# zhizdev/sparsefusion

Hardware: AMD Instinct MI355X
Metric: novel views/sec, distillation steps (2 NGP renders fwd+bwd + VAE enc/dec + 51-eval PLMS + LPIPS), 256^2 / 32x32 latents, 2-view synthetic hydrant (higher is better)
Workload: dtype bf16 MFMA operands / f32 accumulate (UNet); f32 (NGP render)

## Files before the change

include/sparsefusion_hip.h:

```cpp
#ifndef SPARSEFUSION_HIP_H
#define SPARSEFUSION_HIP_H

#include <stdint.h>

#ifdef __cplusplus
extern "C" {
#endif

#define SF_OK 0
#define SF_ERR_INVALID 1
#define SF_ERR_LAUNCH 2

const char* sf_last_error(void);
int sf_abi_version(void);
int sf_operand_is_f16(void);


int sf_grid_encode_forward(const float* inputs, const float* embeddings,
                           const int32_t* offsets, float* outputs,
                           uint32_t B, uint32_t D, uint32_t C, uint32_t L,
                           float S, uint32_t H, float* dy_dx,
                           uint32_t gridtype, int align_corners,
                           const int32_t* h_offsets, void* stream);

// ... 104 lines not shown
int sf_mc_count(const float* vol, uint32_t nx, uint32_t ny, uint32_t nz, float iso,
                void* workspace, uint64_t workspace_bytes, uint32_t* counts2, void* stream);
int sf_mc_emit(const float* vol, uint32_t nx, uint32_t ny, uint32_t nz, float iso,
               void* workspace, uint64_t workspace_bytes, float* verts, int32_t* faces,
               void* stream);

int sf_ngp_render_forward(const sf_ngp_field* f, const float* rays_o,
                          const float* rays_d, const float* aabb, uint32_t N,
                          uint32_t T, float min_near, const float* lin,
                          const float* u_coarse, const float* u_fine,
                          uint32_t u_fine_row_stride, float bg_color, float* nears,
                          float* fars, float* z_sorted, float* sigma_s,
                          float* rgb_s, float* image, float* depth,
                          float* weights_sum, float* field_cache, float* workspace,
                          uint64_t workspace_bytes, void* stream);

int sf_ngp_render_backward(const sf_ngp_field* f, const sf_ngp_field_grad* g,
                           const float* rays_o, const float* rays_d,
                           const float* aabb, uint32_t N, uint32_t T,
                           const float* nears, const float* fars,
                           const float* z_sorted, const float* sigma_s,
                           const float* rgb_s, float bg_color,
                           const float* grad_image, const float* grad_weights_sum,
                           uint32_t rays_per_row, const float* field_cache,
                           float* workspace, uint64_t workspace_bytes,
                           void* stream);

uint64_t sf_ngp_render_workspace_bytes(uint32_t N, uint32_t T);
uint64_t sf_ngp_render_forward_workspace_bytes(uint32_t N, uint32_t T);

uint64_t sf_ngp_render_cache_bytes(uint32_t N, uint32_t T);

int sf_ngp_field_mfma(int on);

int sf_ngp_render_shaded_forward(const sf_ngp_field* f, const float* rays_o, const float* rays_d, const float* aabb,
                                 uint32_t N, uint32_t T, float min_near, const float* lin, const float* u_coarse,
                                 const float* u_fine, uint32_t u_fine_row_stride, float bg_color, const float* light_d,
                                 float ambient_ratio, float epsilon, float* nears, float* fars, float* z_sorted,
                                 float* sigma_s, float* rgb_s, float* normal_s, float* rgb_shaded_s, float* xyz_s,
                                 float* image, float* normal_image, float* orient, float* depth, float* weights_sum,
                                 float* workspace, uint64_t workspace_bytes, void* stream);
uint64_t sf_ngp_render_shaded_workspace_bytes(uint32_t N, uint32_t T);

int sf_ngp_render_occ_eval(const sf_ngp_field* f, const float* rays_o, const float* rays_d,
                           const float* nears, const float* fars, const uint8_t* grid,
                           float dt_gamma, uint32_t max_steps, uint32_t C, uint32_t H,
                           const float* noises, float T_thresh, uint32_t N,
                           float* weights_sum, float* depth, float* image, void* stream);

int sf_ngp_render_occ_eval_shaded(const sf_ngp_field* f, const float* rays_o, const float* rays_d,
        const float* nears, const float* fars, const uint8_t* grid, float dt_gamma, uint32_t max_steps,
        uint32_t C, uint32_t H, const float* noises, float T_thresh, uint32_t N,
        const float* light_d , float ambient_ratio, float epsilon,
        float* weights_sum, float* depth, float* image,
        float* normal_image , uint32_t* n_samples ,
        void* stream);


enum {
  SF_OP_CONV = 1,
  SF_OP_GN_ACT = 2,
  SF_OP_LN = 3,
  SF_OP_GEMV = 4,
  SF_OP_ATTN = 5,
  SF_OP_GCA_POOL = 6,
  SF_OP_ELTWISE = 7,
// ... 81 lines not shown
```

sparsefusion_amd/_lib.py:

```python
import ctypes as C
import os

import torch

_HERE = os.path.dirname(os.path.abspath(__file__))
_DEFAULT_LIB = "libsparsefusion_hip_f16.so" if os.environ.get("SF_OPERAND", "bf16").lower() in ("f16", "fp16", "half") else "libsparsefusion_hip.so"
LIB_PATH = os.environ.get("SF_HIP_LIB") or os.path.join(_HERE, _DEFAULT_LIB)

_lib = None

c_f32p = C.c_void_p
c_i32p = C.c_void_p
u32 = C.c_uint32
u64 = C.c_uint64


class SfNgpField(C.Structure):
    _fields_ = [("embeddings", C.c_void_p), ("h_offsets", C.c_void_p), ("L", u32), ("S", C.c_float),
                ("H", u32), ("gridtype", u32),
                ("w0", C.c_void_p), ("b0", C.c_void_p), ("w1", C.c_void_p), ("b1", C.c_void_p),
                ("w2", C.c_void_p), ("b2", C.c_void_p), ("bound", C.c_float)]


class SfNgpFieldGrad(C.Structure):
# ... 45 lines not shown
                                C.c_void_p, c_f32p, c_f32p, c_f32p, c_f32p, c_f32p, c_f32p, C.c_void_p]),
    "sf_composite_rays": (C.c_int, [u32, u32, C.c_float, c_i32p, c_f32p, c_f32p, c_f32p, c_f32p, c_f32p, c_f32p,
                                    c_f32p, C.c_void_p]),
    "sf_adam_multi": (C.c_int, [C.POINTER(SfAdamArgs), C.c_void_p]),
    "sf_loss_partial_rows": (u32, []),
    "sf_upsample2x_forward": (C.c_int, [c_f32p, c_f32p, u32, u32, u32, C.c_void_p]),
    "sf_upsample2x_backward": (C.c_int, [c_f32p, c_f32p, u32, u32, u32, C.c_void_p]),
    "sf_render_loss_forward": (C.c_int, [c_f32p, c_f32p, c_f32p, c_f32p, u64, u64, C.c_float, c_f32p, C.c_void_p]),
    "sf_render_loss_backward": (C.c_int, [c_f32p, c_f32p, c_f32p, c_f32p, u64, u64, C.c_float, C.c_float, C.c_float, C.c_float,
                                          C.c_float, c_f32p, c_f32p, c_f32p, C.c_void_p]),
    "sf_fusion_loss_forward": (C.c_int, [c_f32p, c_f32p, c_f32p, c_f32p, u32, u64, u64, c_f32p, C.c_void_p]),
    "sf_fusion_loss_backward": (C.c_int, [c_f32p, c_f32p, c_f32p, c_f32p, u32, u64, u64, C.c_float, C.c_float, C.c_float,
                                          c_f32p, c_f32p, c_f32p, C.c_void_p]),
    "sf_ngp_density": (C.c_int, [C.POINTER(SfNgpField), c_f32p, u32, c_f32p, c_f32p, C.c_void_p]),
    "sf_ngp_density_lattice": (C.c_int, [C.POINTER(SfNgpField), c_f32p, c_f32p, c_f32p, u32, u32, u32, c_f32p, C.c_void_p]),
    "sf_ngp_point_attrs": (C.c_int, [C.POINTER(SfNgpField), c_f32p, u32, C.c_float, c_f32p, c_f32p, c_f32p, c_f32p, C.c_void_p]),
    "sf_ngp_texture_bake": (C.c_int, [C.POINTER(SfNgpField), c_f32p, u32, c_i32p, u32, u32, C.c_void_p, c_f32p, c_f32p, c_i32p,
                                      C.c_void_p]),
    "sf_gaussian3d_workspace_bytes": (u64, [u32, u32, u32]),
    "sf_gaussian3d": (C.c_int, [c_f32p, c_f32p, u32, u32, u32, C.c_float, C.c_float, C.c_void_p, C.c_void_p, u64, C.c_void_p]),
    "sf_mc_workspace_bytes": (u64, [u32, u32, u32]),
    "sf_mc_count": (C.c_int, [c_f32p, u32, u32, u32, C.c_float, C.c_void_p, u64, C.c_void_p, C.c_void_p]),
    "sf_mc_emit": (C.c_int, [c_f32p, u32, u32, u32, C.c_float, C.c_void_p, u64, c_f32p, c_i32p, C.c_void_p]),
    "sf_ngp_render_forward": (C.c_int, [C.POINTER(SfNgpField), c_f32p, c_f32p, c_f32p, u32, u32, C.c_float,
                                        c_f32p, c_f32p, c_f32p, u32, C.c_float, c_f32p, c_f32p, c_f32p, c_f32p,
                                        c_f32p, c_f32p, c_f32p, c_f32p, c_f32p, c_f32p, u64, C.c_void_p]),
    "sf_ngp_render_backward": (C.c_int, [C.POINTER(SfNgpField), C.POINTER(SfNgpFieldGrad), c_f32p, c_f32p,
                                         c_f32p, u32, u32, c_f32p, c_f32p, c_f32p, c_f32p, c_f32p,
                                         C.c_float, c_f32p, c_f32p, u32, c_f32p, c_f32p, u64, C.c_void_p]),
    "sf_ngp_render_workspace_bytes": (u64, [u32, u32]),
    "sf_ngp_render_forward_workspace_bytes": (u64, [u32, u32]),
    "sf_ngp_render_cache_bytes": (u64, [u32, u32]),
    "sf_ngp_field_mfma": (C.c_int, [C.c_int]),
    "sf_ngp_render_shaded_forward": (C.c_int, [C.POINTER(SfNgpField), c_f32p, c_f32p, c_f32p, u32, u32, C.c_float, c_f32p, c_f32p,
                                               c_f32p, u32, C.c_float, c_f32p, C.c_float, C.c_float, c_f32p, c_f32p, c_f32p,
                                               c_f32p, c_f32p, c_f32p, c_f32p, c_f32p, c_f32p, c_f32p, c_f32p, c_f32p, c_f32p,
                                               c_f32p, u64, C.c_void_p]),
    "sf_ngp_render_shaded_workspace_bytes": (u64, [u32, u32]),
    "sf_ngp_render_occ_eval": (C.c_int, [C.POINTER(SfNgpField), c_f32p, c_f32p, c_f32p, c_f32p, C.c_void_p, C.c_float, u32, u32, u32,
                                         c_f32p, C.c_float, u32, c_f32p, c_f32p, c_f32p, C.c_void_p]),
    "sf_ngp_render_occ_eval_shaded": (C.c_int, [C.POINTER(SfNgpField), c_f32p, c_f32p, c_f32p, c_f32p, C.c_void_p, C.c_float, u32, u32,
                                                u32, c_f32p, C.c_float, u32, c_f32p, C.c_float, C.c_float, c_f32p, c_f32p, c_f32p,
                                                c_f32p, C.c_void_p, C.c_void_p]),
    "sf_plan_run": (C.c_int, [C.POINTER(SfOp), u32, C.c_void_p]),
    "sf_conv_igemm_t_launches": (u64, []),
    "sf_gca4_launches": (u64, [C.c_int]),
    "sf_plan_profile": (C.c_int, [C.POINTER(SfOp), u32, C.c_void_p, C.c_void_p]),
    "sf_conv_packed_elems": (u64, [u32, u32, u32, u32]),
    "sf_conv_pack_weights": (C.c_int, [C.c_void_p, u32, u32, u32, u32, u32, C.c_void_p]),
    "sf_plms_update": (C.c_int, [c_f32p, c_f32p, c_f32p, C.c_void_p, u64, c_f32p, c_f32p, C.c_void_p]),
    "sf_plms_combine": (C.c_int, [c_f32p, c_f32p, c_f32p, c_f32p, C.c_void_p, u64, c_f32p, c_f32p, C.c_void_p]),
    "sf_plms_step": (C.c_int, [c_f32p, c_f32p, c_f32p, c_f32p, C.c_void_p, c_f32p, c_f32p, c_f32p, C.c_void_p, u64, c_f32p, c_f32p, c_f32p, u64, C.c_void_p]),
}


_handles = {}


def _load(path):
    if path not in _handles:
        if not os.path.exists(path):
            raise RuntimeError(
                f"{path} is missing: build it with `python -m sparsefusion_amd.build` (`--f16` for the IEEE-half operand build; "
                "there is no CPU fallback for the sparsefusion_amd hot path)")
        handle = C.CDLL(path)
        for name, (res, args) in SIGNATURES.items():
# ... 43 lines not shown
```

sparsefusion_amd/csrc/ngp_render.hip:

```cpp

#include "sf_common.h"
#include "ngp_device.h"
#include "ngp_field_lds.h"
#include "ngp_bwd_mfma.h"
#include "ngp_field_mfma.h"
#include "ngp_composite_wave.h"
#include "ngp_scatter_bin.h"
#include "ngp_shade.h"
#include <stdlib.h>
#include <atomic>
#include <mutex>

struct GridLevels;
int sf_fill_levels(GridLevels* lv, const int32_t* offsets_dev, const int32_t* h_offsets, uint32_t L, float S,
                   uint32_t H, hipStream_t st);

template <int MODE>
__global__ __launch_bounds__(256) void k_ngp_field(
    FieldPtrs f, NgpLevels lv, const float* __restrict__ rays_o, const float* __restrict__ rays_d,
    const float* __restrict__ aabb, const float* __restrict__ nears, const float* __restrict__ fars,
    const float* __restrict__ lin, const float* __restrict__ u, const float* __restrict__ z_in,
    const float* __restrict__ xyz_in, uint32_t P, uint32_t T, float* __restrict__ z_out,
    float* __restrict__ sigma, float* __restrict__ rgb, float* __restrict__ feat_out = nullptr) {
  __shared__ __attribute__((aligned(16))) float W[NGP_WTOTAL];
  load_weights_lds(W, f);
  __syncthreads();
  float box[6];
  if (MODE != 2) {
#pragma unroll
    for (int i = 0; i < 6; ++i) box[i] = aabb[i];
  }
  for (uint32_t p = blockIdx.x * blockDim.x + threadIdx.x; p < P; p += gridDim.x * blockDim.x) {
    asm volatile("" ::: "memory");
    float x[3];
    if (MODE == 2) {
      x[0] = xyz_in[p * 3 + 0]; x[1] = xyz_in[p * 3 + 1]; x[2] = xyz_in[p * 3 + 2];
    } else {
// ... 246 lines not shown
    uint32_t per = 8192;
    if ((N + per - 1) / per > 64) per = (((N + 63) / 64 + 255) / 256) * 256;
    c.n = (N + per - 1) / per; c.max_rays = per;
    for (uint32_t i = 0; i < c.n; ++i) c.start[i] = i * per;
    c.start[c.n] = N;
    return c;
  }
  equal(k);
  return c;
}
#define SB_CURSOR_WORDS (NGP_MAX_LEVELS * SB_MAX_BUCKETS)
#ifndef SB_LEVELS_BUDGET
#define SB_LEVELS_BUDGET 24
#endif
static uint64_t ngp_bin_entries(uint32_t N, uint32_t T) {
  return (uint64_t)ngp_bwd_plan(N).max_rays * 2 * T * 4 * SB_LEVELS_BUDGET + (uint64_t)SB_CURSOR_WORDS * 64;
}
extern "C" uint64_t sf_ngp_render_workspace_bytes(uint32_t N, uint32_t T) {
  return (uint64_t)(8 + 4 * NGP_MAX_LEVELS) * N * T * sizeof(float) + (uint64_t)SB_CURSOR_WORDS * 4 + ngp_bin_entries(N, T) * 16;
}

extern "C" uint64_t sf_ngp_render_forward_workspace_bytes(uint32_t N, uint32_t T) { return (uint64_t)10 * N * T * sizeof(float); }

#ifndef FM_GRID_CAP
#define FM_GRID_CAP 512u
#endif
static std::atomic<int> g_field_mfma{1};
extern "C" int sf_ngp_field_mfma(int on) {
  const int was = g_field_mfma.load(std::memory_order_relaxed);
  if (on >= 0) g_field_mfma.store(on ? 1 : 0, std::memory_order_relaxed);
  return was;
}

extern "C" uint64_t sf_ngp_render_cache_bytes(uint32_t N, uint32_t T) {
  return ((uint64_t)2 * N * T * NGP_FEAT + (uint64_t)N * 2 * T) * sizeof(float);
}

extern "C" int sf_ngp_render_forward(const sf_ngp_field* f, const float* rays_o, const float* rays_d,
                                     const float* aabb, uint32_t N, uint32_t T, float min_near,
                                     const float* lin, const float* u_coarse, const float* u_fine,
                                     uint32_t u_fine_row_stride, float bg_color, float* nears, float* fars,
                                     float* z_sorted, float* sigma_s, float* rgb_s, float* image, float* depth,
                                     float* weights_sum, float* field_cache, float* workspace, uint64_t workspace_bytes,
                                     void* stream) {
  hipStream_t st = (hipStream_t)stream;
  if (N == 0) return SF_OK;
  if (T < 4 || T > 64) SF_FAIL(SF_ERR_INVALID, "ngp_render: T must be in [4,64]");
  if (workspace_bytes < sf_ngp_render_forward_workspace_bytes(N, T)) SF_FAIL(SF_ERR_INVALID, "ngp_render: workspace too small");
  if (!lin || !u_fine) SF_FAIL(SF_ERR_INVALID, "ngp_render: lin and u_fine tables are required");
  NgpLevels lv;
  if (int rc = sf_ngp_make_levels(f, &lv, st)) return rc;
  if (int rc = sf_near_far_from_aabb(rays_o, rays_d, aabb, N, min_near, nears, fars, stream)) return rc;
  const uint64_t NT = (uint64_t)N * T;
  float* z_c = workspace;           float* sig_c = z_c + NT;     float* rgb_c = sig_c + NT;
  float* z_f = rgb_c + 3 * NT;      float* sig_f = z_f + NT;     float* rgb_f = sig_f + NT;
  const FieldPtrs fp = field_ptrs(f);
  const uint32_t P = (uint32_t)NT;
  const uint32_t gridp = sf_grid_cap(sf_div_up(P, 256));
  float* feat_c = field_cache;
  float* feat_f = field_cache ? field_cache + NT * NGP_FEAT : nullptr;
  uint32_t* perm = field_cache ? reinterpret_cast<uint32_t*>(field_cache + 2 * NT * NGP_FEAT) : nullptr;
  const bool mfma = g_field_mfma.load(std::memory_order_relaxed) != 0;
  FMArgs fm{};
  fm.table = fp.table; fm.w0 = fp.w0; fm.b0 = fp.b0; fm.w1 = fp.w1; fm.b1 = fp.b1; fm.w2 = fp.w2; fm.b2 = fp.b2; fm.bound = fp.bound;
  fm.lv = lv; fm.rays_o = rays_o; fm.rays_d = rays_d; fm.aabb = aabb; fm.nears = nears; fm.fars = fars; fm.P = P; fm.T = T;
  const uint32_t gridm = sf_div_up(sf_div_up(P, FM_PTS), 4) < FM_GRID_CAP ? sf_div_up(sf_div_up(P, FM_PTS), 4) : FM_GRID_CAP;
// ... 106 lines not shown
      props.allocType = hipMemAllocationTypePinned;
      props.location.type = hipMemLocationTypeDevice;
      props.location.id = dev_id;
      hipMemPool_t np = nullptr;
      uint64_t keep = UINT64_MAX;
      if (hipMemPoolCreate(&np, &props) != hipSuccess) SF_FAIL(SF_ERR_LAUNCH, "ngp_render_backward: cannot create the scratch pool");
      if (hipMemPoolSetAttribute(np, hipMemPoolAttrReleaseThreshold, &keep) != hipSuccess) {
        (void)hipMemPoolDestroy(np);
        SF_FAIL(SF_ERR_LAUNCH, "ngp_render_backward: cannot configure the scratch pool");
      }
      pools[dev_id] = np;
    }
    pool = pools[dev_id];
  }
  struct FixBuf {
    long long* p = nullptr; hipStream_t st = nullptr;
    ~FixBuf() { if (p) (void)hipFreeAsync(p, st); }
  } fix;
  fix.st = st;
  const uint64_t fix_bytes = segs.end[FIX_SEGS - 1] * sizeof(long long);
  const hipError_t alloc = pool ? hipMallocFromPoolAsync(reinterpret_cast<void**>(&fix.p), fix_bytes, pool, st)
                               : hipMallocAsync(reinterpret_cast<void**>(&fix.p), fix_bytes, st);
  if (alloc != hipSuccess || !fix.p)
    SF_FAIL(SF_ERR_LAUNCH, "ngp_render_backward: cannot allocate the gradient accumulators");
  if (hipMemsetAsync(fix.p, 0, fix_bytes, st) != hipSuccess) SF_FAIL(SF_ERR_LAUNCH, "ngp_render_backward: memset failed");
  long long* acc_tab = fix.p;
  long long* acc_mlp = fix.p + tab_n;
  const float thr_tab = sf_fix_thr(8.0 * (double)M);
  const size_t lds2 = (size_t)FB_LDS_FLOATS * sizeof(float);
  const size_t lds_sc = (size_t)SC_SLOTS * (sizeof(uint32_t) + 2 * sizeof(long long));
  static unsigned attr_mask = 0;
  if (dev_id >= 32 || !(attr_mask & (1u << dev_id))) {
    if (hipFuncSetAttribute(reinterpret_cast<const void*>(&k_ngp_field_bwd_mfma), hipFuncAttributeMaxDynamicSharedMemorySize, (int)lds2) != hipSuccess ||
        hipFuncSetAttribute(reinterpret_cast<const void*>(&k_ngp_scatter<1024>), hipFuncAttributeMaxDynamicSharedMemorySize, (int)lds_sc) != hipSuccess)
      SF_FAIL(SF_ERR_LAUNCH, "ngp_render_backward: cannot raise the dynamic LDS limits");
    if (dev_id < 32) attr_mask |= 1u << dev_id;
  }
  constexpr float sc_cutoff = 640.0f;
#ifndef SC_RUN
#define SC_RUN 32u
#endif
  constexpr uint32_t sc_run = SC_RUN;
  uint32_t cached = 0;
  while (cached < lv.L && lv.scale[cached] <= sc_cutoff) ++cached;
  constexpr float bin_cutoff = 60.0f;
  uint32_t first_bin = lv.L;
  uint32_t bucket0[NGP_MAX_LEVELS + 1] = {};
  if (dfeat) {
    first_bin = 0;
    while (first_bin < lv.L && lv.scale[first_bin] <= bin_cutoff) ++first_bin;
    uint32_t tb = 0;
    for (uint32_t l = 0; l <= NGP_MAX_LEVELS; ++l) {
      bucket0[l] = tb;
      if (l >= first_bin && l < lv.L) {
        const uint32_t nb = (lv.hsize[l] + SB_ROWS - 1) >> SB_ROWS_LOG;
        if (nb > SB_MAX_BUCKETS) { first_bin = lv.L; break; }
        tb += nb;
      }
    }
  }
  const bool binned = first_bin < lv.L;
  if (binned && cached > first_bin) cached = first_bin;
  const uint32_t last = !dfeat ? lv.L : binned ? first_bin : cached;
  const uint32_t total_buckets = bucket0[NGP_MAX_LEVELS];
  uint32_t* bin_cursor = reinterpret_cast<uint32_t*>(workspace + (size_t)(8 + 4 * NGP_MAX_LEVELS) * N * T);
  f32x4* bin_ent = reinterpret_cast<f32x4*>(bin_cursor + SB_CURSOR_WORDS);
// ... 12 lines not shown
  std::unique_lock<std::mutex> side_lk(side_mu, std::defer_lock);
  struct SideJoin {
    Side* sd = nullptr; hipStream_t st = nullptr; bool forked = false;
    int join() { const bool f = forked; forked = false; return (!f || (hipEventRecord(sd->join, sd->s) == hipSuccess && hipStreamWaitEvent(st, sd->join, 0) == hipSuccess)) ? 0 : 1; }
    ~SideJoin() { (void)join(); }
  } side_join;
  if (fork) {
    side_lk.lock();
    Side& sd = side[dev_id];
    if (!sd.s && (hipStreamCreateWithFlags(&sd.s, hipStreamNonBlocking) != hipSuccess ||
                  hipEventCreateWithFlags(&sd.fork, hipEventDisableTiming) != hipSuccess ||
                  hipEventCreateWithFlags(&sd.join, hipEventDisableTiming) != hipSuccess))
      SF_FAIL(SF_ERR_LAUNCH, "ngp_render_backward: cannot create the side stream");
    side_join.sd = &sd; side_join.st = st;
  }
  const uint32_t T2 = 2 * T;
  for (uint32_t c = 0; c < n_chunks; ++c) {
    const uint32_t n0 = plan.start[c], Nc = plan.start[c + 1] - n0;
    const uint32_t Pc = Nc * T2, P0 = n0 * T2;
    FBArgs a{};
    a.table = f->embeddings; a.w0 = f->w0; a.b0 = f->b0; a.w1 = f->w1; a.b1 = f->b1; a.w2 = f->w2; a.b2 = f->b2; a.bound = f->bound;
    a.g_w0 = acc_mlp + (segs.end[0] - tab_n); a.g_b0 = acc_mlp + (segs.end[1] - tab_n); a.g_w1 = acc_mlp + (segs.end[2] - tab_n);
    a.g_b1 = acc_mlp + (segs.end[3] - tab_n); a.g_w2 = acc_mlp + (segs.end[4] - tab_n); a.g_b2 = acc_mlp + (segs.end[5] - tab_n);
    a.f_w0 = g->g_w0; a.f_b0 = g->g_b0; a.f_w1 = g->g_w1; a.f_b1 = g->g_b1; a.f_w2 = g->g_w2; a.f_b2 = g->g_b2; a.thr = thr_mlp;
    a.lv = lv;
    a.rays_o = rays_o + (size_t)n0 * 3; a.rays_d = rays_d + (size_t)n0 * 3; a.aabb = aabb;
    a.z_s = z_sorted + (size_t)P0; a.dsig = dsig + (size_t)P0; a.drgb = drgb + (size_t)P0 * 3; a.dfeat_out = dfeat;
    a.P = Pc; a.T2 = T2; a.dfeat_P = (uint32_t)M; a.p_off = P0;
    a.feat_c = field_cache;
    a.feat_f = field_cache ? field_cache + (size_t)N * T * NGP_FEAT : nullptr;
    a.perm = field_cache ? reinterpret_cast<const uint32_t*>(field_cache + 2 * (size_t)N * T * NGP_FEAT) : nullptr;
    const uint32_t trips = sf_div_up(Pc, FB_PTS);
    const uint32_t grid = trips < 1024 ? sf_div_up(trips, 4) : 256;
    k_ngp_field_bwd_mfma<<<grid, 256, lds2, st>>>(a);
    SF_CHECK_LAUNCH("ngp_field_bwd_mfma");
    if (dfeat && last < lv.L) {
      hipStream_t sf = st;
      if (fork) {
        Side& sd = side[dev_id];
        if (hipEventRecord(sd.fork, st) != hipSuccess || hipStreamWaitEvent(sd.s, sd.fork, 0) != hipSuccess)
          SF_FAIL(SF_ERR_LAUNCH, "ngp_render_backward: fork failed");
        sf = sd.s;
        side_join.forked = true;
      }
      if (binned) {
        SBArgs b{};
        b.lv = lv; b.bound = f->bound; b.rays_o = a.rays_o; b.rays_d = a.rays_d; b.aabb = aabb; b.z_s = a.z_s; b.dfeat = dfeat;
        b.gtable = acc_tab; b.gtable_f = g->g_embeddings; b.thr = thr_tab; b.cursor = bin_cursor; b.ent = bin_ent;
        b.P = Pc; b.T2 = T2; b.first_level = first_bin; b.P_stride = (uint32_t)M; b.p_off = P0; b.cap = bin_cap;
        SBRArgs r{};
        r.lv = lv; r.gtable = acc_tab; r.gtable_f = g->g_embeddings; r.thr = thr_tab; r.cursor = bin_cursor; r.ent = bin_ent; r.first_level = first_bin; r.cap = bin_cap;
        for (uint32_t l = 0; l <= NGP_MAX_LEVELS; ++l) { b.bucket0[l] = bucket0[l]; r.bucket0[l] = bucket0[l]; }
        const uint32_t tiles = sf_div_up(Pc, SB_THREADS);
        k_ngp_bin<<<tiles < 1024 ? tiles : 1024, SB_THREADS, 0, sf>>>(b);
        SF_CHECK_LAUNCH("ngp_bin");
        k_ngp_bin_reduce<<<total_buckets, SBR_THREADS, 0, sf>>>(r);
        SF_CHECK_LAUNCH("ngp_bin_reduce");
      } else {
        const uint64_t items = (uint64_t)4 * Pc * (lv.L - last);
        const uint32_t grid_f = (uint32_t)(items / 256 < 16384 ? (items + 255) / 256 : 16384);
        k_ngp_scatter_fine<<<grid_f, 256, 0, sf>>>(lv, f->bound, acc_tab, g->g_embeddings, thr_tab, a.rays_o, a.rays_d, aabb, a.z_s, dfeat, Nc, T2, last,
                                                   (uint32_t)M, P0);
        SF_CHECK_LAUNCH("ngp_scatter_fine");
      }
    }
  }
  if (dfeat && last > 0) {
    const uint32_t grid_sc = sf_div_up(N, SC_RAYS);
// ... 13 lines not shown
```

sparsefusion_amd/nerf/renderer.py:

```python
import argparse
import ctypes as C
import math
import os

import torch
import torch.nn as nn

from .. import _lib
from .utils import safe_normalize


def get_default_torch_ngp_opt():
    opt = argparse.Namespace()
    opt.cuda_ray = False
    opt.max_steps = 256
    opt.num_steps = 64
    opt.upsample_steps = 64
    opt.update_extra_interval = 16
    opt.max_ray_batch = 4096
    opt.albedo_iters = 1000
    opt.bg_radius = 0
    opt.density_thresh = 10
    opt.fp16 = True
    opt.backbone = 'grid'
# ... 6 lines not shown
    opt.lambda_entropy = 1e-4
    opt.lambda_opacity = 0
    opt.lambda_orient = 1e-2
    opt.lambda_smooth = 0
    return opt


class _FieldHandle:

    def __init__(self, net):
        enc = net.encoder
        lin = net.sigma_net.net
        self.tensors = [enc.embeddings, lin[0].weight, lin[0].bias, lin[1].weight, lin[1].bias, lin[2].weight,
                        lin[2].bias]
        self.host_offsets = enc.host_offsets
        self.L = enc.num_levels
        self.S = float(math.log2(enc.per_level_scale))
        self.H = int(enc.base_resolution)
        self.gridtype = int(enc.gridtype_id)
        self.bound = float(net.bound)

    def struct(self, tensors):
        f = _lib.SfNgpField()
        f.embeddings = tensors[0].data_ptr()
        f.h_offsets = self.host_offsets.ctypes.data
        f.L, f.S, f.H, f.gridtype = self.L, self.S, self.H, self.gridtype
        f.w0, f.b0, f.w1, f.b1, f.w2, f.b2 = (t.data_ptr() for t in tensors[1:])
        f.bound = self.bound
        return f


_FEAT_CACHE = True
_FIELD_MFMA = True


def _select_field_kernel(lib):
    lib.sf_ngp_field_mfma(1 if _FIELD_MFMA else 0)


class _RenderFn(torch.autograd.Function):
    @staticmethod
    def forward(ctx, handle, rays_o, rays_d, aabb, T, min_near, lin, u_coarse, u_fine, u_stride, bg, rays_per_row, grad_mode, *params):
        _lib.require_cuda(rays_o, rays_d, aabb, *params)
        params = [p.detach().contiguous() for p in params]
        N = rays_o.shape[0]
        dev = rays_o.device
        f32 = dict(dtype=torch.float32, device=dev)
        nears, fars = torch.empty(N, **f32), torch.empty(N, **f32)
        z_s, sig_s = torch.empty(N, 2 * T, **f32), torch.empty(N, 2 * T, **f32)
        rgb_s = torch.empty(N, 2 * T, 3, **f32)
        image, depth, ws = torch.empty(N, 3, **f32), torch.empty(N, **f32), torch.empty(N, **f32)
        lib = _lib.lib()
        wbytes = lib.sf_ngp_render_forward_workspace_bytes(N, T)
        work = torch.empty(max(1, wbytes // 4), **f32)
        f = handle.struct(params)
        cache = None
        if _FEAT_CACHE and grad_mode and any(ctx.needs_input_grad[13:]):
            cache = torch.empty(lib.sf_ngp_render_cache_bytes(N, T) // 4, **f32)
        _select_field_kernel(lib)
        rc = lib.sf_ngp_render_forward(C.byref(f), _lib.ptr(rays_o), _lib.ptr(rays_d), _lib.ptr(aabb), N, T,
                                       float(min_near), _lib.ptr(lin), _lib.ptr(u_coarse), _lib.ptr(u_fine),
                                       int(u_stride), float(bg), _lib.ptr(nears), _lib.ptr(fars), _lib.ptr(z_s),
                                       _lib.ptr(sig_s), _lib.ptr(rgb_s), _lib.ptr(image), _lib.ptr(depth), _lib.ptr(ws),
                                       _lib.ptr(cache), _lib.ptr(work), wbytes, _lib.stream_ptr())
        _lib.check(rc, "ngp_render_forward")
        ctx.handle, ctx.T, ctx.bg, ctx.rays_per_row = handle, T, float(bg), int(rays_per_row)
        ctx.has_cache = cache is not None
        ctx.save_for_backward(rays_o, rays_d, aabb, nears, fars, z_s, sig_s, rgb_s, *([cache] if cache is not None else []), *params)
        ctx.mark_non_differentiable(depth, nears, fars)
        return image, ws, depth, nears, fars

    @staticmethod
    def backward(ctx, g_image, g_ws, _gd, _gn, _gf):
        rays_o, rays_d, aabb, nears, fars, z_s, sig_s, rgb_s, *params = ctx.saved_tensors
        cache = params.pop(0) if ctx.has_cache else None
        N, T = rays_o.shape[0], ctx.T
        grads = [torch.zeros_like(p) for p in params]
        g = _lib.SfNgpFieldGrad()
        (g.g_embeddings, g.g_w0, g.g_b0, g.g_w1, g.g_b1, g.g_w2, g.g_b2) = (t.data_ptr() for t in grads)
        f = ctx.handle.struct(params)
        lib = _lib.lib()
        wbytes = lib.sf_ngp_render_workspace_bytes(N, T)
        work = torch.empty(max(1, wbytes // 4), dtype=torch.float32, device=rays_o.device)
        g_image = (g_image if g_image is not None else torch.zeros(N, 3, device=rays_o.device)).contiguous().float()
        g_ws = g_ws.contiguous().float() if g_ws is not None else None
        rc = lib.sf_ngp_render_backward(C.byref(f), C.byref(g), _lib.ptr(rays_o), _lib.ptr(rays_d), _lib.ptr(aabb), N, T,
                                        _lib.ptr(nears), _lib.ptr(fars), _lib.ptr(z_s), _lib.ptr(sig_s), _lib.ptr(rgb_s),
                                        ctx.bg, _lib.ptr(g_image), _lib.ptr(g_ws), int(ctx.rays_per_row), _lib.ptr(cache),
                                        _lib.ptr(work), wbytes, _lib.stream_ptr())
        _lib.check(rc, "ngp_render_backward")
        return (None,) * 13 + tuple(grads)


class NeRFRenderer(nn.Module):
    def __init__(self, opt):
        super().__init__()
        self.opt = opt
        self.bound = opt.bound
        self.cascade = 1 + math.ceil(math.log2(opt.bound))
        self.grid_size = 128
        self.cuda_ray = opt.cuda_ray
        self.min_near = opt.min_near
        self.density_thresh = opt.density_thresh
        self.bg_radius = opt.bg_radius
        if self.bg_radius > 0:
            raise NotImplementedError("bg_radius > 0 is not on the distillation path (distillation.py:512)")
        box = torch.tensor([-opt.bound] * 3 + [opt.bound] * 3, dtype=torch.float32)
        self.register_buffer('aabb_train', box)
        self.register_buffer('aabb_infer', box.clone())
        self._tables = {}
        if self.cuda_ray:
            self.register_buffer('density_grid', torch.zeros([self.cascade, self.grid_size ** 3]))
            self.register_buffer('density_bitfield', torch.zeros(self.cascade * self.grid_size ** 3 // 8, dtype=torch.uint8))
            self.mean_density = 0
            self.iter_density = 0
            self.register_buffer('step_counter', torch.zeros(16, 2, dtype=torch.int32))
            self.mean_count = 0
            self.local_step = 0
# ... 321 lines not shown
```

Baseline: 18.29.

## Add software-pipelined NGP field backward kernel with prefetch and register-resident weights

Result: faster. 18.52 (median of 6 runs) (+1.2%).

```diff
diff --git a/include/sparsefusion_hip.h b/include/sparsefusion_hip.h
--- a/include/sparsefusion_hip.h
+++ b/include/sparsefusion_hip.h
@@ -160,6 +160,9 @@
 uint64_t sf_ngp_render_cache_bytes(uint32_t N, uint32_t T);
 
 int sf_ngp_field_mfma(int on);
+
+int sf_ngp_field_bwd_pipe(int on);
+void sf_ngp_field_bwd_launches(uint64_t* counts);
 
 int sf_ngp_render_shaded_forward(const sf_ngp_field* f, const float* rays_o, const float* rays_d, const float* aabb,
                                  uint32_t N, uint32_t T, float min_near, const float* lin, const float* u_coarse,
diff --git a/sparsefusion_amd/_lib.py b/sparsefusion_amd/_lib.py
--- a/sparsefusion_amd/_lib.py
+++ b/sparsefusion_amd/_lib.py
@@ -101,6 +101,8 @@
     "sf_ngp_render_forward_workspace_bytes": (u64, [u32, u32]),
     "sf_ngp_render_cache_bytes": (u64, [u32, u32]),
     "sf_ngp_field_mfma": (C.c_int, [C.c_int]),
+    "sf_ngp_field_bwd_pipe": (C.c_int, [C.c_int]),
+    "sf_ngp_field_bwd_launches": (None, [C.c_void_p]),
     "sf_ngp_render_shaded_forward": (C.c_int, [C.POINTER(SfNgpField), c_f32p, c_f32p, c_f32p, u32, u32, C.c_float, c_f32p, c_f32p,
                                                c_f32p, u32, C.c_float, c_f32p, C.c_float, C.c_float, c_f32p, c_f32p, c_f32p,
                                                c_f32p, c_f32p, c_f32p, c_f32p, c_f32p, c_f32p, c_f32p, c_f32p, c_f32p, c_f32p,
diff --git a/sparsefusion_amd/csrc/ngp_bwd_pipe.h b/sparsefusion_amd/csrc/ngp_bwd_pipe.h
--- /dev/null
+++ b/sparsefusion_amd/csrc/ngp_bwd_pipe.h
@@ -0,0 +1,433 @@
+#pragma once
+#include "ngp_bwd_mfma.h"
+
+#ifndef SF_FIELD_BWD_PIPE_DEFAULT
+#define SF_FIELD_BWD_PIPE_DEFAULT 1
+#endif
+#ifndef FP_W1_REGS
+#define FP_W1_REGS 1
+#endif
+#ifndef FP_H1_REGS
+#define FP_H1_REGS 1
+#endif
+#ifndef FP_PREFETCH
+#define FP_PREFETCH 1
+#endif
+
+struct FPOps {
+  f32x4 fv[4];
+  float z, o[3], d[3];
+  float g0, g1;
+};
+
+SF_DEV void fp_load(const FBArgs& a, uint32_t pc, uint32_t src, int half, FPOps& q) {
+  const uint32_t pg = a.p_off + pc, ng = pg / a.T2, T = a.T2 >> 1, n = pc / a.T2;
+  const float* row = (src < T ? a.feat_c + ((size_t)ng * T + src) * NGP_FEAT : a.feat_f + ((size_t)ng * T + (src - T)) * NGP_FEAT) + half * 16;
+#pragma unroll
+  for (int j = 0; j < 4; ++j) q.fv[j] = *reinterpret_cast<const f32x4*>(row + 4 * j);
+  q.z = a.z_s[pc];
+#pragma unroll
+  for (int i = 0; i < 3; ++i) { q.o[i] = a.rays_o[n * 3 + i]; q.d[i] = a.rays_d[n * 3 + i]; }
+  q.g0 = half == 0 ? a.dsig[pc] : a.drgb[(size_t)pc * 3 + 1];
+  q.g1 = half == 0 ? a.drgb[(size_t)pc * 3] : a.drgb[(size_t)pc * 3 + 2];
+}
+
+SF_KERNEL(256) void k_ngp_field_bwd_pipe(FBArgs a) {
+  SF_DYN_LDS(lds_raw);
+  float* W = reinterpret_cast<float*>(lds_raw);
+  const int tid = threadIdx.x, lane = tid & 63, wave = tid >> 6;
+  float* F = W + FB_WTOT + wave * FB_WAVE_FLOATS;
+  float* H1 = F + FB_PTS * FB_SF;
+  float* H2 = H1 + FB_PTS * FB_SH;
+  float* DO = H2 + FB_PTS * FB_SH;
+  float* INS = DO + FB_PTS * 4;
+  for (int i = tid; i < NGP_HID * NGP_FEAT; i += 256) W[FB_W0 + (i >> 5) * FB_SF + (i & 31)] = a.w0[i];
+  for (int i = tid; i < NGP_HID * NGP_HID; i += 256) W[FB_W1 + (i >> 6) * FB_SH + (i & 63)] = a.w1[i];
+  for (int i = tid; i < NGP_OUT * NGP_HID; i += 256) W[FB_W2 + i] = a.w2[i];
+  if (tid < NGP_HID) { W[FB_B0 + tid] = a.b0[tid]; W[FB_B1 + tid] = a.b1[tid]; }
+  if (tid < NGP_OUT) W[FB_B2 + tid] = a.b2[tid];
+  float box[6];
+#pragma unroll
+  for (int i = 0; i < 6; ++i) box[i] = a.aabb[i];
+  sf_sync();
+
+  const int li = lane & 15, kq = lane >> 4;
+  const int pl = lane & 31, half = lane >> 5;
+#if FP_W1_REGS >= 1
+  float bw1[NGP_HID / 4][4];
+#pragma unroll
+  for (int s = 0; s < NGP_HID / 4; ++s)
+#pragma unroll
+    for (int nt = 0; nt < 4; ++nt) bw1[s][nt] = W[FB_W1 + (nt * 16 + li) * FB_SH + 4 * s + kq];
+#endif
+#if FP_W1_REGS >= 2
+  float gw1[NGP_HID / 4][4];
+#pragma unroll
+  for (int s = 0; s < NGP_HID / 4; ++s)
+#pragma unroll
+    for (int nt = 0; nt < 4; ++nt) gw1[s][nt] = W[FB_W1 + (4 * s + kq) * FB_SH + nt * 16 + li];
+#endif
+  float cw2[NGP_HID / 4], ew2[4], bb0[4], bb1[4];
+#pragma unroll
+  for (int s = 0; s < NGP_HID / 4; ++s) {
+    const float v = W[FB_W2 + (li & 3) * NGP_HID + 4 * s + kq];
+    cw2[s] = li < NGP_OUT ? v : 0.0f;
+  }
+#pragma unroll
+  for (int nt = 0; nt < 4; ++nt) {
+    ew2[nt] = W[FB_W2 + kq * NGP_HID + nt * 16 + li];
+    bb0[nt] = W[FB_B0 + nt * 16 + li];
+    bb1[nt] = W[FB_B1 + nt * 16 + li];
+  }
+  const float cb2 = li < NGP_OUT ? W[FB_B2 + (li & 3)] : 0.0f;
+
+  f32x4 acc1[4][4], acc0[4][2];
+  f32x4 acc2[4], accb2 = f32x4{0.f, 0.f, 0.f, 0.f};
+#pragma unroll
+  for (int i = 0; i < 4; ++i) {
+#pragma unroll
+    for (int j = 0; j < 4; ++j) acc1[i][j] = f32x4{0.f, 0.f, 0.f, 0.f};
+    acc0[i][0] = f32x4{0.f, 0.f, 0.f, 0.f};
+    acc0[i][1] = f32x4{0.f, 0.f, 0.f, 0.f};
+    acc2[i] = f32x4{0.f, 0.f, 0.f, 0.f};
+  }
+  float accb1 = 0.0f, accb0 = 0.0f;
+
+  const uint32_t n_trips = (a.P + FB_PTS - 1) / FB_PTS, stride = gridDim.x * 4;
+  uint32_t trip = blockIdx.x * 4 + wave;
+#define FP_POINT(t) ((t) < n_trips && (t) * FB_PTS + pl < a.P ? (t) * FB_PTS + pl : a.P - 1)
+#if FP_PREFETCH
+  FPOps cur;
+  uint32_t perm_nxt = 0;
+  if (trip < n_trips) {
+    const uint32_t pc = FP_POINT(trip);
+    fp_load(a, pc, a.perm[a.p_off + pc], half, cur);
+    perm_nxt = a.perm[a.p_off + FP_POINT(trip + stride)];
+  }
+#endif
+  for (; trip < n_trips; trip += stride) {
+    const uint32_t p0 = trip * FB_PTS;
+    const uint32_t p = p0 + pl;
+    const bool live = p < a.P;
+#if FP_PREFETCH
+    FPOps nxt;
+    fp_load(a, FP_POINT(trip + stride), perm_nxt, half, nxt);
+    const uint32_t perm_nn = a.perm[a.p_off + FP_POINT(trip + 2 * stride)];
+#else
+    FPOps cur;
+    {
+      const uint32_t pc = FP_POINT(trip);
+      fp_load(a, pc, a.perm[a.p_off + pc], half, cur);
+    }
+#endif
+    float x[3] = {0.f, 0.f, 0.f}, x01[3] = {0.f, 0.f, 0.f};
+    bool inside = false;
+    if (live) {
+      ngp_point(cur.o, cur.d, cur.z, box, x);
+      inside = ngp_unit(x, a.bound, x01);
+    }
+#pragma unroll
+    for (int j = 0; j < 4; ++j)
+#pragma unroll
+      for (int e = 0; e < 4; ++e) F[pl * FB_SF + half * 16 + 4 * j + e] = live ? cur.fv[j][e] : 0.0f;
+    if (half == 0) INS[pl] = inside ? 1.0f : 0.0f;
+    sf_wave_sync();
+
+    f32x4 h1r[2][4], h2r[2][4];
+    {
+      float av[2][NGP_FEAT / 4], bv[NGP_FEAT / 4][4];
+#pragma unroll
+      for (int s = 0; s < NGP_FEAT / 4; ++s) {
+        av[0][s] = F[li * FB_SF + 4 * s + kq];
+        av[1][s] = F[(16 + li) * FB_SF + 4 * s + kq];
+#pragma unroll
+        for (int nt = 0; nt < 4; ++nt) bv[s][nt] = W[FB_W0 + (nt * 16 + li) * FB_SF + 4 * s + kq];
+      }
+#pragma unroll
+      for (int nt = 0; nt < 4; ++nt) { h1r[0][nt] = f32x4{bb0[nt], bb0[nt], bb0[nt], bb0[nt]}; h1r[1][nt] = h1r[0][nt]; }
+#pragma unroll
+      for (int s = 0; s < NGP_FEAT / 4; ++s)
+#pragma unroll
+        for (int nt = 0; nt < 4; ++nt) {
+          h1r[0][nt] = sf_mfma4(av[0][s], bv[s][nt], h1r[0][nt]);
+          h1r[1][nt] = sf_mfma4(av[1][s], bv[s][nt], h1r[1][nt]);
+        }
+#pragma unroll
+      for (int mt = 0; mt < 2; ++mt)
+#pragma unroll
+        for (int nt = 0; nt < 4; ++nt)
+#pragma unroll
+          for (int r = 0; r < 4; ++r) {
+            h1r[mt][nt][r] = fmaxf(h1r[mt][nt][r], 0.0f);
+            H1[(mt * 16 + 4 * kq + r) * FB_SH + nt * 16 + li] = h1r[mt][nt][r];
+          }
+    }
+    sf_wave_sync();
+    {
+      float av[2][NGP_HID / 4];
+#pragma unroll
+      for (int s = 0; s < NGP_HID / 4; ++s) {
+        av[0][s] = H1[li * FB_SH + 4 * s + kq];
+        av[1][s] = H1[(16 + li) * FB_SH + 4 * s + kq];
+      }
+#pragma unroll
+      for (int nt = 0; nt < 4; ++nt) { h2r[0][nt] = f32x4{bb1[nt], bb1[nt], bb1[nt], bb1[nt]}; h2r[1][nt] = h2r[0][nt]; }
+#pragma unroll
+      for (int s = 0; s < NGP_HID / 4; ++s)
+#pragma unroll
+        for (int nt = 0; nt < 4; ++nt) {
+#if FP_W1_REGS >= 1
+          const float b = bw1[s][nt];
+#else
+          const float b = W[FB_W1 + (nt * 16 + li) * FB_SH + 4 * s + kq];
+#endif
+          h2r[0][nt] = sf_mfma4(av[0][s], b, h2r[0][nt]);
+          h2r[1][nt] = sf_mfma4(av[1][s], b, h2r[1][nt]);
+        }
+#pragma unroll
+      for (int mt = 0; mt < 2; ++mt)
+#pragma unroll
+        for (int nt = 0; nt < 4; ++nt)
+#pragma unroll
+          for (int r = 0; r < 4; ++r) {
+            h2r[mt][nt][r] = fmaxf(h2r[mt][nt][r], 0.0f);
+            H2[(mt * 16 + 4 * kq + r) * FB_SH + nt * 16 + li] = h2r[mt][nt][r];
+          }
+    }
+    sf_wave_sync();
+    {
+      float av[2][NGP_HID / 4];
+#pragma unroll
+      for (int s = 0; s < NGP_HID / 4; ++s) {
+        av[0][s] = H2[li * FB_SH + 4 * s + kq];
+        av[1][s] = H2[(16 + li) * FB_SH + 4 * s + kq];
+      }
+      f32x4 c[2];
+      c[0] = f32x4{cb2, cb2, cb2, cb2};
+      c[1] = c[0];
+#pragma unroll
+      for (int s = 0; s < NGP_HID / 4; ++s) {
+        c[0] = sf_mfma4(av[0][s], cw2[s], c[0]);
+        c[1] = sf_mfma4(av[1][s], cw2[s], c[1]);
+      }
+      if (li < NGP_OUT) {
+#pragma unroll
+        for (int mt = 0; mt < 2; ++mt)
+#pragma unroll
+          for (int r = 0; r < 4; ++r) DO[(mt * 16 + 4 * kq + r) * 4 + li] = c[mt][r];
+      }
+      sf_wave_sync();
+      const float o0 = DO[pl * 4 + 2 * half], o1 = DO[pl * 4 + 2 * half + 1];
+      float d0 = 0.0f, d1 = 0.0f;
+      if (live) {
+        if (half == 0) {
+          const float pre = o0 + ngp_blob(x);
+          d0 = cur.g0 * expf(fminf(fmaxf(pre, -15.0f), 15.0f));
+          const float sg = ngp_sigmoid(o1);
+          d1 = cur.g1 * sg * (1.0f - sg);
+        } else {
+          const float s0 = ngp_sigmoid(o0), s1 = ngp_sigmoid(o1);
+          d0 = cur.g0 * s0 * (1.0f - s0);
+          d1 = cur.g1 * s1 * (1.0f - s1);
+        }
+      }
+      DO[pl * 4 + 2 * half] = d0;
+      DO[pl * 4 + 2 * half + 1] = d1;
+    }
+    sf_wave_sync();
+    {
+      float da[FB_PTS / 4], hb[FB_PTS / 4][4], ea[2];
+#pragma unroll
+      for (int s = 0; s < FB_PTS / 4; ++s) {
+        const float v = DO[(4 * s + kq) * 4 + (li & 3)];
+        da[s] = li < NGP_OUT ? v : 0.0f;
+#pragma unroll
+        for (int kt = 0; kt < 4; ++kt) hb[s][kt] = H2[(4 * s + kq) * FB_SH + kt * 16 + li];
+      }
+      ea[0] = DO[li * 4 + kq];
+      ea[1] = DO[(16 + li) * 4 + kq];
+      f32x4 b = f32x4{0.f, 0.f, 0.f, 0.f};
+#pragma unroll
+      for (int s = 0; s < FB_PTS / 4; ++s) {
+#pragma unroll
+        for (int kt = 0; kt < 4; ++kt) acc2[kt] = sf_mfma4(da[s], hb[s][kt], acc2[kt]);
+        b = sf_mfma4(da[s], 1.0f, b);
+      }
+#pragma unroll
+      for (int r = 0; r < 4; ++r) accb2[r] += b[r];
+      sf_wave_sync();
+#pragma unroll
+      for (int mt = 0; mt < 2; ++mt)
+#pragma unroll
+        for (int nt = 0; nt < 4; ++nt) {
+          const f32x4 g = sf_mfma4(ea[mt], ew2[nt], f32x4{0.f, 0.f, 0.f, 0.f});
+#pragma unroll
+          for (int r = 0; r < 4; ++r) H2[(mt * 16 + 4 * kq + r) * FB_SH + nt * 16 + li] = h2r[mt][nt][r] > 0.0f ? g[r] : 0.0f;
+        }
+    }
+    sf_wave_sync();
+    {
+      float b = 0.0f;
+#pragma unroll
+      for (int hs = 0; hs < 2; ++hs) {
+        float av[FB_PTS / 8][4], bv[FB_PTS / 8][4], col[FB_PTS / 2];
+#pragma unroll
+        for (int s = 0; s < FB_PTS / 8; ++s)
+#pragma unroll
+          for (int t = 0; t < 4; ++t) {
+            av[s][t] = H2[(16 * hs + 4 * s + kq) * FB_SH + t * 16 + li];
+            bv[s][t] = H1[(16 * hs + 4 * s + kq) * FB_SH + t * 16 + li];
+          }
+#pragma unroll
+        for (int q = 0; q < FB_PTS / 2; ++q) col[q] = H2[(16 * hs + q) * FB_SH + lane];
+#pragma unroll
+        for (int s = 0; s < FB_PTS / 8; ++s)
+#pragma unroll
+          for (int jt = 0; jt < 4; ++jt)
+#pragma unroll
+            for (int kt = 0; kt < 4; ++kt) acc1[jt][kt] = sf_mfma4(av[s][jt], bv[s][kt], acc1[jt][kt]);
+#pragma unroll
+        for (int q = 0; q < FB_PTS / 2; ++q) b += col[q];
+      }
+      accb1 += b;
+    }
+    {
+      float av[2][NGP_HID / 4];
+#pragma unroll
+      for (int s = 0; s < NGP_HID / 4; ++s) {
+        av[0][s] = H2[li * FB_SH + 4 * s + kq];
+        av[1][s] = H2[(16 + li) * FB_SH + 4 * s + kq];
+      }
+      f32x4 c[2][4];
+#pragma unroll
+      for (int nt = 0; nt < 4; ++nt) { c[0][nt] = f32x4{0.f, 0.f, 0.f, 0.f}; c[1][nt] = c[0][nt]; }
+#pragma unroll
+      for (int s = 0; s < NGP_HID / 4; ++s)
+#pragma unroll
+        for (int nt = 0; nt < 4; ++nt) {
+#if FP_W1_REGS >= 2
+          const float b = gw1[s][nt];
+#else
+          const float b = W[FB_W1 + (4 * s + kq) * FB_SH + nt * 16 + li];
+#endif
+          c[0][nt] = sf_mfma4(av[0][s], b, c[0][nt]);
+          c[1][nt] = sf_mfma4(av[1][s], b, c[1][nt]);
+        }
+      sf_wave_sync();
+#pragma unroll
+      for (int mt = 0; mt < 2; ++mt)
+#pragma unroll
+        for (int nt = 0; nt < 4; ++nt)
+#pragma unroll
+          for (int r = 0; r < 4; ++r) {
+            float* hp = H1 + (mt * 16 + 4 * kq + r) * FB_SH + nt * 16 + li;
+#if FP_H1_REGS
+            *hp = h1r[mt][nt][r] > 0.0f ? c[mt][nt][r] : 0.0f;
+#else
+            *hp = *hp > 0.0f ? c[mt][nt][r] : 0.0f;
+#endif
+          }
+    }
+    sf_wave_sync();
+    {
+      float av[FB_PTS / 4][4], bv[FB_PTS / 4][2], col[FB_PTS];
+#pragma unroll
+      for (int s = 0; s < FB_PTS / 4; ++s) {
+#pragma unroll
+        for (int t = 0; t < 4; ++t) av[s][t] = H1[(4 * s + kq) * FB_SH + t * 16 + li];
+        bv[s][0] = F[(4 * s + kq) * FB_SF + li];
+        bv[s][1] = F[(4 * s + kq) * FB_SF + 16 + li];
+      }
+#pragma unroll
+      for (int q = 0; q < FB_PTS; ++q) col[q] = H1[q * FB_SH + lane];
+#pragma unroll
+      for (int s = 0; s < FB_PTS / 4; ++s)
+#pragma unroll
+        for (int jt = 0; jt < 4; ++jt) {
+          acc0[jt][0] = sf_mfma4(av[s][jt], bv[s][0], acc0[jt][0]);
+          acc0[jt][1] = sf_mfma4(av[s][jt], bv[s][1], acc0[jt][1]);
+        }
+      float b = 0.0f;
+#pragma unroll
+      for (int q = 0; q < FB_PTS; ++q) b += col[q];
+      accb0 += b;
+    }
+    if (a.dfeat_out) {
+      float av[2][NGP_HID / 4], bv[NGP_HID / 4][2];
+#pragma unroll
+      for (int s = 0; s < NGP_HID / 4; ++s) {
+        av[0][s] = H1[li * FB_SH + 4 * s + kq];
+        av[1][s] = H1[(16 + li) * FB_SH + 4 * s + kq];
+        bv[s][0] = W[FB_W0 + (4 * s + kq) * FB_SF + li];
+        bv[s][1] = W[FB_W0 + (4 * s + kq) * FB_SF + 16 + li];
+      }
+      f32x4 c[2][2];
+      c[0][0] = c[0][1] = c[1][0] = c[1][1] = f32x4{0.f, 0.f, 0.f, 0.f};
+#pragma unroll
+      for (int s = 0; s < NGP_HID / 4; ++s) {
+        c[0][0] = sf_mfma4(av[0][s], bv[s][0], c[0][0]);
+        c[0][1] = sf_mfma4(av[0][s], bv[s][1], c[0][1]);
+        c[1][0] = sf_mfma4(av[1][s], bv[s][0], c[1][0]);
+        c[1][1] = sf_mfma4(av[1][s], bv[s][1], c[1][1]);
+      }
+      sf_wave_sync();
+#pragma unroll
+      for (int mt = 0; mt < 2; ++mt)
+#pragma unroll
+        for (int ft = 0; ft < 2; ++ft)
+#pragma unroll
+          for (int r = 0; r < 4; ++r) {
+            const int q = mt * 16 + 4 * kq + r, f = ft * 16 + li;
+            F[q * FB_SF + f] = INS[q] != 0.0f ? c[mt][ft][r] : 0.0f;
+          }
+      sf_wave_sync();
+      {
+        const uint32_t l = lane >> 2, q0 = (lane & 3) * 8;
+        if (l < a.lv.L) {
+          float* dst = a.dfeat_out + ((size_t)l * a.dfeat_P + a.p_off + p0 + q0) * 2;
+          if (p0 + FB_PTS <= a.P && !((a.dfeat_P | a.p_off) & 1)) {
+#pragma unroll
+            for (int j = 0; j < 4; ++j) {
+              f32x4 v;
+              v[0] = F[(q0 + 2 * j) * FB_SF + 2 * l];     v[1] = F[(q0 + 2 * j) * FB_SF + 2 * l + 1];
+              v[2] = F[(q0 + 2 * j + 1) * FB_SF + 2 * l]; v[3] = F[(q0 + 2 * j + 1) * FB_SF + 2 * l + 1];
+              *reinterpret_cast<f32x4*>(dst + 4 * j) = v;
+            }
+          } else {
+            for (int j = 0; j < 8; ++j)
+              if (p0 + q0 + j < a.P) { dst[2 * j] = F[(q0 + j) * FB_SF + 2 * l]; dst[2 * j + 1] = F[(q0 + j) * FB_SF + 2 * l + 1]; }
+          }
+        }
+      }
+    }
+    sf_wave_sync();
+#if FP_PREFETCH
+    cur = nxt;
+    perm_nxt = perm_nn;
+#endif
+  }
+#undef FP_POINT
+
+#pragma unroll
+  for (int jt = 0; jt < 4; ++jt)
+#pragma unroll
+    for (int r = 0; r < 4; ++r) {
+      const int j = jt * 16 + 4 * kq + r;
+#pragma unroll
+      for (int kt = 0; kt < 4; ++kt) sf_grad_add(a.g_w1 + j * NGP_HID + kt * 16 + li, a.f_w1 + j * NGP_HID + kt * 16 + li, acc1[jt][kt][r], a.thr);
+      sf_grad_add(a.g_w0 + j * NGP_FEAT + li, a.f_w0 + j * NGP_FEAT + li, acc0[jt][0][r], a.thr);
+      sf_grad_add(a.g_w0 + j * NGP_FEAT + 16 + li, a.f_w0 + j * NGP_FEAT + 16 + li, acc0[jt][1][r], a.thr);
+    }
+  if (kq == 0) {
+#pragma unroll
+    for (int kt = 0; kt < 4; ++kt)
+#pragma unroll
+      for (int r = 0; r < 4; ++r) sf_grad_add(a.g_w2 + r * NGP_HID + kt * 16 + li, a.f_w2 + r * NGP_HID + kt * 16 + li, acc2[kt][r], a.thr);
+    if (li == 0) {
+#pragma unroll
+      for (int r = 0; r < 4; ++r) sf_grad_add(a.g_b2 + r, a.f_b2 + r, accb2[r], a.thr);
+    }
+  }
+  sf_grad_add(a.g_b1 + lane, a.f_b1 + lane, accb1, a.thr);
+  sf_grad_add(a.g_b0 + lane, a.f_b0 + lane, accb0, a.thr);
+}
diff --git a/sparsefusion_amd/csrc/ngp_render.hip b/sparsefusion_amd/csrc/ngp_render.hip
--- a/sparsefusion_amd/csrc/ngp_render.hip
+++ b/sparsefusion_amd/csrc/ngp_render.hip
@@ -3,6 +3,7 @@
 #include "ngp_device.h"
 #include "ngp_field_lds.h"
 #include "ngp_bwd_mfma.h"
+#include "ngp_bwd_pipe.h"
 #include "ngp_field_mfma.h"
 #include "ngp_composite_wave.h"
 #include "ngp_scatter_bin.h"
@@ -315,6 +316,18 @@
   return was;
 }
 
+static std::atomic<int> g_field_bwd_pipe{SF_FIELD_BWD_PIPE_DEFAULT};
+static std::atomic<uint64_t> g_field_bwd_launches[2];
+extern "C" int sf_ngp_field_bwd_pipe(int on) {
+  const int was = g_field_bwd_pipe.load(std::memory_order_relaxed);
+  if (on >= 0) g_field_bwd_pipe.store(on ? 1 : 0, std::memory_order_relaxed);
+  return was;
+}
+extern "C" void sf_ngp_field_bwd_launches(uint64_t* counts) {
+  counts[0] = g_field_bwd_launches[0].load(std::memory_order_relaxed);
+  counts[1] = g_field_bwd_launches[1].load(std::memory_order_relaxed);
+}
+
 extern "C" uint64_t sf_ngp_render_cache_bytes(uint32_t N, uint32_t T) {
   return ((uint64_t)2 * N * T * NGP_FEAT + (uint64_t)N * 2 * T) * sizeof(float);
 }
@@ -487,6 +500,7 @@
   static unsigned attr_mask = 0;
   if (dev_id >= 32 || !(attr_mask & (1u << dev_id))) {
     if (hipFuncSetAttribute(reinterpret_cast<const void*>(&k_ngp_field_bwd_mfma), hipFuncAttributeMaxDynamicSharedMemorySize, (int)lds2) != hipSuccess ||
+        hipFuncSetAttribute(reinterpret_cast<const void*>(&k_ngp_field_bwd_pipe), hipFuncAttributeMaxDynamicSharedMemorySize, (int)lds2) != hipSuccess ||
         hipFuncSetAttribute(reinterpret_cast<const void*>(&k_ngp_scatter<1024>), hipFuncAttributeMaxDynamicSharedMemorySize, (int)lds_sc) != hipSuccess)
       SF_FAIL(SF_ERR_LAUNCH, "ngp_render_backward: cannot raise the dynamic LDS limits");
     if (dev_id < 32) attr_mask |= 1u << dev_id;
@@ -565,8 +579,11 @@
     a.perm = field_cache ? reinterpret_cast<const uint32_t*>(field_cache + 2 * (size_t)N * T * NGP_FEAT) : nullptr;
     const uint32_t trips = sf_div_up(Pc, FB_PTS);
     const uint32_t grid = trips < 1024 ? sf_div_up(trips, 4) : 256;
-    k_ngp_field_bwd_mfma<<<grid, 256, lds2, st>>>(a);
-    SF_CHECK_LAUNCH("ngp_field_bwd_mfma");
+    const int pipe = field_cache && g_field_bwd_pipe.load(std::memory_order_relaxed) != 0 ? 1 : 0;
+    if (pipe) k_ngp_field_bwd_pipe<<<grid, 256, lds2, st>>>(a);
+    else k_ngp_field_bwd_mfma<<<grid, 256, lds2, st>>>(a);
+    SF_CHECK_LAUNCH(pipe ? "ngp_field_bwd_pipe" : "ngp_field_bwd_mfma");
+    g_field_bwd_launches[pipe].fetch_add(1, std::memory_order_relaxed);
     if (dfeat && last < lv.L) {
       hipStream_t sf = st;
       if (fork) {
diff --git a/sparsefusion_amd/nerf/renderer.py b/sparsefusion_amd/nerf/renderer.py
--- a/sparsefusion_amd/nerf/renderer.py
+++ b/sparsefusion_amd/nerf/renderer.py
@@ -62,10 +62,15 @@
 
 _FEAT_CACHE = True
 _FIELD_MFMA = True
+_FIELD_BWD_PIPE = True
 
 
 def _select_field_kernel(lib):
     lib.sf_ngp_field_mfma(1 if _FIELD_MFMA else 0)
+
+
+def _select_field_bwd_kernel(lib):
+    lib.sf_ngp_field_bwd_pipe(1 if _FIELD_BWD_PIPE else 0)
 
 
 class _RenderFn(torch.autograd.Function):
@@ -114,6 +119,7 @@
         work = torch.empty(max(1, wbytes // 4), dtype=torch.float32, device=rays_o.device)
         g_image = (g_image if g_image is not None else torch.zeros(N, 3, device=rays_o.device)).contiguous().float()
         g_ws = g_ws.contiguous().float() if g_ws is not None else None
+        _select_field_bwd_kernel(lib)
         rc = lib.sf_ngp_render_backward(C.byref(f), C.byref(g), _lib.ptr(rays_o), _lib.ptr(rays_d), _lib.ptr(aabb), N, T,
                                         _lib.ptr(nears), _lib.ptr(fars), _lib.ptr(z_s), _lib.ptr(sig_s), _lib.ptr(rgb_s),
                                         ctx.bg, _lib.ptr(g_image), _lib.ptr(g_ws), int(ctx.rays_per_row), _lib.ptr(cache),
```
